# nevi-me/rust-dataframe

Measured on AMD Instinct MI355X. Metric: rows/sec filter+sum over 1e9 f64 Arrow rows; %HBM bw at 1/2/4/8 GPU, higher is better.
Workload: dtype f64

## Files before the change

rust_dataframe_amd/csrc/rdf_capi.cpp:

```cpp
#include <hip/hip_runtime.h>

#include <algorithm>
#include <cmath>
#include <cstdarg>
#include <cstdio>
#include <chrono>
#include <functional>
#include <cstring>
#include <map>
#include <memory>
#include <mutex>
#include <condition_variable>
#include <string>
#include <thread>
#include <vector>
#include <sys/syscall.h>
#include <unistd.h>

#include "rdf_device.h"
#include "rdf_stage_copy.h"

using namespace rdfk;

namespace {
// ... 54 lines not shown
    int    opt_gb_hot = 1;
    int    opt_gb_bucket = 0;
    int    opt_gb_partition = 3;
    bool   timing = false;
    std::vector<std::pair<hipEvent_t, hipEvent_t>> events;
    size_t events_used = 0;
    std::multimap<size_t, void*> pool_free;
    size_t pool_cached = 0;
    int64_t opt_stream_slab = 0;
    void*  sbuf_dev[2] = {nullptr, nullptr};
    void*  sbuf_pin[2] = {nullptr, nullptr};
    size_t sbuf_dev_cap = 0, sbuf_pin_cap = 0;
    hipEvent_t sbuf_ev[2] = {nullptr, nullptr};
    void*  dbuf_dev[2] = {nullptr, nullptr};
    void*  dbuf_pin[2] = {nullptr, nullptr};
    size_t dbuf_dev_cap = 0, dbuf_pin_cap = 0;
    hipEvent_t dbuf_ev[2] = {nullptr, nullptr};
    hipStream_t d2h_stream = nullptr;
    int64_t stream_slabs = 0, stream_bytes_staged = 0, stream_bytes_direct = 0;
    bool in_stream = false;
    bool streaming = false;
    int  opt_stream_table_kernel = 1;
    char* tab_pin = nullptr; size_t tab_pin_cap = 0, tab_pin_used = 0;
    bool   agg_comm_entered = false;
    ::rdf_comm* agg_comm = nullptr;
    ~Ctx();
};

thread_local Ctx g_ctx;

Ctx::~Ctx() {
    if (!ready || (long)syscall(SYS_gettid) == (long)getpid()) return;
    (void)hipSetDevice(device);
    if (stream) (void)hipStreamSynchronize(stream);
    for (void* p : arena.overflow) (void)hipFree(p);
    if (arena.base) (void)hipFree(arena.base);
    if (pinned) (void)hipHostFree(pinned);
    for (auto& kv : pool_free) (void)hipFree(kv.second);
    for (int b = 0; b < 2; ++b) { if (sbuf_dev[b]) (void)hipFree(sbuf_dev[b]); if (sbuf_pin[b]) (void)hipHostFree(sbuf_pin[b]); if (sbuf_ev[b]) (void)hipEventDestroy(sbuf_ev[b]); }
    if (tab_pin) (void)hipHostFree(tab_pin);
    if (d2h_stream) (void)hipStreamSynchronize(d2h_stream);
    for (int b = 0; b < 2; ++b) { if (dbuf_dev[b]) (void)hipFree(dbuf_dev[b]); if (dbuf_pin[b]) (void)hipHostFree(dbuf_pin[b]); if (dbuf_ev[b]) (void)hipEventDestroy(dbuf_ev[b]); }
    if (d2h_stream) (void)hipStreamDestroy(d2h_stream);
    for (auto& ev : events) { (void)hipEventDestroy(ev.first); (void)hipEventDestroy(ev.second); }
    if (copy_stream) { (void)hipStreamSynchronize(copy_stream); (void)hipStreamDestroy(copy_stream); }
    if (own_stream) (void)hipStreamDestroy(own_stream);
    ready = false;
}

rdf_status fail(rdf_status st, const char* fmt, ...) {
    char buf[512];
    va_list ap;
    va_start(ap, fmt);
    vsnprintf(buf, sizeof buf, fmt, ap);
    va_end(ap);
    g_ctx.err = buf;
    if (g_ctx.ready && g_ctx.stream) (void)hipStreamSynchronize(g_ctx.stream);
    return st;
}

// ... 834 lines not shown
                    static const int mir[6] = {LH_F_LT, LH_F_LE, LH_F_EQ, LH_F_NE, LH_F_GT, LH_F_GE};
                    h = (sw ? mir : fwd)[op - RDF_OP_GT];
                } else if (op == RDF_OP_AND) h = LH_AND;
                else if (op == RDF_OP_OR) h = LH_OR;
                else if (in.dtype == RDF_F64) {
                    if (op == RDF_OP_ADD) h = LH_F_ADD;
                    else if (op == RDF_OP_MUL) h = LH_F_MUL;
                    else if (op == RDF_OP_SUB) h = sw ? LH_F_RSUB : LH_F_SUB;
                    else if (op == RDF_OP_DIV) h = sw ? LH_F_RDIV : LH_F_DIV;
                } else if (in.dtype == RDF_I64 || in.dtype == RDF_U64) {
                    if (op == RDF_OP_ADD) h = LH_I_ADD;
                    else if (op == RDF_OP_MUL) h = LH_I_MUL;
                    else if (op == RDF_OP_SUB) h = sw ? LH_I_RSUB : LH_I_SUB;
                }
            } break;
            default: break;
        }
        if (h == LH_NONE) return false;
        lean.code[i].swapped = (uint8_t)((in.swapped & 1) | (h << 1));
    }
    return true;
}

rdf_status launch_agg_pair(const EvalArgs* ea, const FilterAggF64Args* fa, int cmp, int feat, int grid, int nvalues,
                           const int* cls, AggPartial* partials, AggPartial* result, const char* spec_sig = nullptr,
                           const SpecArgs* sa = nullptr) {
    Ctx& c = g_ctx;
    KernelTimer kt;
    if (sa) {
        const bool jit = jit_find(spec_sig) != nullptr;
        c.last_kernel = std::string("spec_kernel<") + spec_sig + ">" + (jit ? " [compiled at run time]" : "");
        const hipError_t le = launch_spec(spec_sig, *sa, grid, c.stream);
        if (le != hipSuccess && jit) { (void)hipGetLastError(); return kRetryInterpreted; }
        if (le != hipSuccess) return fail(RDF_DEVICE_ERROR, "launch_spec: %s", hipGetErrorString(le));
    }
    else if (fa) { c.last_kernel = "filter_agg_f64_kernel"; HIP_TRY(launch_filter_agg_f64(*fa, cmp, grid, c.stream)); }
    else {
        EvalArgs lean;
        if (c.opt_interp_lean && feat == 0 && lean_assign(*ea, lean)) { c.last_kernel = "eval_kernel<AGG, lean>"; HIP_TRY(launch_eval_lean(lean, SINK_AGG, grid, c.stream, c.opt_interp_lean == 2)); }
        else { c.last_kernel = "eval_kernel<AGG>"; HIP_TRY(launch_eval(*ea, SINK_AGG, feat, grid, c.stream)); }
    }
    kt.stop();
    AggFinalArgs f;
    memset(&f, 0, sizeof f);
    f.partials = partials;
    f.result = result;
    f.nblocks = grid;
    f.nvalues = nvalues;
    for (int k = 0; k < nvalues; ++k) f.value_cls[k] = cls[k];
    HIP_TRY(launch_agg_final(f, c.stream));
    return RDF_OK;
}

void fill_agg_result(rdf_agg_result* r, int dt, const AggPartial& p) {
    memset(r, 0, sizeof *r);
    r->dtype = dt;
    r->count = p.cnt;
    r->is_some = p.cnt > 0;
    if (is_float(dt)) {
        double s, a, b;
        memcpy(&s, &p.sum, 8); memcpy(&a, &p.mn, 8); memcpy(&b, &p.mx, 8);
        r->sum_f64 = dt == RDF_F32 ? (double)(float)s : s;
        if (p.cnt > 0) { r->min_f64 = a; r->max_f64 = b; }
    } else {
        r->sum_i64 = (int64_t)h_normalize_int(dt, p.sum);
        if (p.cnt > 0) { r->min_i64 = (int64_t)p.mn; r->max_i64 = (int64_t)p.mx; }
    }
}

}

struct rdf_frame {
    int device = 0;
// ... 285 lines not shown
            for (size_t i = 0; i < dev_outs.size(); ++i) dev_outs[i] = DevOutChunk{outs[i].values, outs[i].validity};
        }
    }

    std::vector<int64_t> tile_start;
    const rdf_frame::Tiles* eval_tiles = nullptr;
    if (fc) RDF_TRY(frame_tiles(*fc, kEvalTile, &eval_tiles));
    else {
        tile_start.assign((size_t)nchunks + 1, 0);
        for (int64_t c = 0; c < nchunks; ++c) tile_start[(size_t)c + 1] = tile_start[(size_t)c] + (clen[(size_t)c] + kEvalTile - 1) / kEvalTile;
    }
    const int64_t ntiles = fc ? eval_tiles->ntiles : tile_start[(size_t)nchunks];
    int grid = (int)(ntiles < (int64_t)eval_grid_limit() ? ntiles : (int64_t)eval_grid_limit());

    const size_t n_nc = ps.sink == RDF_SINK_STORE ? (size_t)ps.nvalues * (size_t)nchunks : 0;
    const int gwords = grouped ? group_words(ps.ngroups, ps.nvalues) : 0;
    const size_t scratch_bytes = 16 + n_nc * 8 + ((size_t)grid + 4) * (grouped ? (size_t)gwords * 8 : (size_t)ps.nvalues * sizeof(AggPartial));
    void* scratch = nullptr;
    RDF_TRY(arena_alloc(scratch_bytes, &scratch));
    uint32_t* d_flags = (uint32_t*)scratch;
    int64_t* d_nullc = (int64_t*)((char*)scratch + 16);
    AggPartial* d_partials = (AggPartial*)((char*)scratch + 16 + n_nc * 8);
    AggPartial* d_result = d_partials + (size_t)grid * (size_t)ps.nvalues;
    HIP_TRY(hipMemsetAsync(scratch, 0, 16 + n_nc * 8, ctx.stream));

    EvalArgs ea;
    memset(&ea, 0, sizeof ea);
    ea.nchunks = nchunks;
    ea.ntiles = ntiles;
    ea.ncols = ncols;
    ea.nvalues = ps.nvalues;
    ea.ncode = (int)cc.code.size();
    ea.ntmp = cc.tmp_max;
    ea.flags = d_flags;
    ea.out_null_counts = d_nullc;
    ea.partials = d_partials;
    for (int k = 0; k < ncols; ++k) ea.col_dtype[k] = col_dtype[k];
    int cls[kMaxGroupValues] = {0, 0, 0, 0, 0, 0, 0, 0};
    for (int v = 0; v < ps.nvalues; ++v) { cls[v] = value_class(value_dtype[v]); ea.value_cls[v] = cls[v]; }
    memcpy(ea.code, cc.code.data(), cc.code.size() * sizeof(Instr));

    TableBuilder tb;
    auto build_eval_tables = [&]() -> rdf_status {
        if (nchunks == 1) {
            for (int k = 0; k < ncols; ++k) ea.inline_cols[k] = in_dev[(size_t)k];
            for (int v = 0; v < ps.nvalues && ps.sink == RDF_SINK_STORE; ++v) ea.inline_outs[v] = dev_outs[(size_t)v];
            ea.inline_len = clen[0];
// ... 262 lines not shown
                if (L.kind == RDF_NODE_COLUMN && R.kind == RDF_NODE_SCALAR) { coln = &L; sc = &R; }
                else if (L.kind == RDF_NODE_SCALAR && R.kind == RDF_NODE_COLUMN) {
                    coln = &R; sc = &L;
                    cmp = fr.op == RDF_OP_GT ? RDF_OP_LT : fr.op == RDF_OP_GE ? RDF_OP_LE : fr.op == RDF_OP_LT ? RDF_OP_GT : fr.op == RDF_OP_LE ? RDF_OP_GE : fr.op;
                }
                if (coln && col_dtype[coln->column] == RDF_F64 && sc->dtype != RDF_NULLTYPE && (is_numeric(sc->dtype) || sc->dtype == RDF_BOOL)) {
                    const DevChunkCol& x = in_dev[(size_t)coln->column];
                    const DevChunkCol& y = in_dev[(size_t)vr.column];
                    const uintptr_t xa = (uintptr_t)((const double*)x.values + x.offset), ya = (uintptr_t)((const double*)y.values + y.offset);
                    if ((xa & 7) == 0 && (ya & 7) == 0 && (xa & 15) == (ya & 15)) {
                        memset(&fa, 0, sizeof fa);
                        fa.x = (const double*)x.values; fa.x_validity = x.validity; fa.x_offset = x.offset;
                        fa.y = (const double*)y.values; fa.y_validity = y.validity; fa.y_offset = y.offset;
                        fa.n = clen[0];
                        const uint64_t cu = cc.imm_for(*sc, RDF_F64);
                        memcpy(&fa.c, &cu, 8);
                        fa.partials = d_partials;
                        fast = true;
                    }
                }
            }
        }
        if (use_spec) {
            const rdf_status ls = launch_agg_pair(nullptr, nullptr, 0, 0, grid, ps.nvalues, cls, d_partials, d_result, sp.sig.c_str(), &sa);
            if (ls == kRetryInterpreted) return run_program(ps, cols, ncols, nchunks, outs, aggs, len_mismatch_msg, fc);
            RDF_TRY(ls);
        } else if (fast) {
            const int64_t per_block = (int64_t)kBlock * 4 * 2;
            int64_t want = (clen[0] + per_block - 1) / per_block;
            grid = (int)(want < (int64_t)eval_grid_limit() ? want : (int64_t)eval_grid_limit());
            if (grid < 1) grid = 1;
            d_result = d_partials + (size_t)grid * (size_t)ps.nvalues;
            RDF_TRY(launch_agg_pair(nullptr, &fa, cmp, 0, grid, 1, cls, d_partials, d_result));
        } else {
            RDF_TRY(launch_agg_pair(&ea, nullptr, 0, cc.feat(), grid, ps.nvalues, cls, d_partials, d_result));
        }
        if (ctx.agg_comm) {
            AggPartial hp[kMaxValues];
            uint32_t flags = 0;
            RDF_TRY(agg_dist_finish(*ctx.agg_comm, d_result, d_flags, ps.nvalues, cls, hp, &flags));
            if (flags & 2u) return fail(RDF_COMPUTE_ERROR, "pipeline_dist: another rank failed before the combine");
            if (flags & 1u) return fail(RDF_DIVIDE_BY_ZERO, "Divide by zero error");
            for (int v = 0; v < ps.nvalues; ++v) fill_agg_result(&aggs[v], value_dtype[v], hp[v]);
            return RDF_OK;
        }
        RDF_TRY(pinned_reserve(pin_off + 64 + sizeof(AggPartial) * kMaxValues));
        char* pin = ctx.pinned + pin_off;
        HIP_TRY(hipMemcpyAsync(pin, d_flags, 16, hipMemcpyDeviceToHost, ctx.stream));
        HIP_TRY(hipMemcpyAsync(pin + 64, d_result, sizeof(AggPartial) * (size_t)ps.nvalues, hipMemcpyDeviceToHost, ctx.stream));
        HIP_TRY(hipStreamSynchronize(ctx.stream));
        dbg.mark("kernel + result");
        uint32_t flags;
        memcpy(&flags, pin, 4);
        if (flags & 1u) return fail(RDF_DIVIDE_BY_ZERO, "Divide by zero error");
        for (int v = 0; v < ps.nvalues; ++v) {
            AggPartial p;
            memcpy(&p, pin + 64 + sizeof(AggPartial) * (size_t)v, sizeof p);
            fill_agg_result(&aggs[v], value_dtype[v], p);
        }
        return RDF_OK;
    }

    {
        KernelTimer kt;
        if (use_spec) {
            const bool jit = jit_find(sp.sig.c_str()) != nullptr;
            ctx.last_kernel = "spec_kernel<" + sp.sig + ">" + (jit ? " [compiled at run time]" : "");
            const hipError_t le = launch_spec(sp.sig.c_str(), sa, grid, ctx.stream);
            if (le != hipSuccess && jit) { (void)hipGetLastError(); return run_program(ps, cols, ncols, nchunks, outs, aggs, len_mismatch_msg, fc); }
            if (le != hipSuccess) return fail(RDF_DEVICE_ERROR, "launch_spec: %s", hipGetErrorString(le));
        }
        else {
            int64_t longest = 0;
            for (int64_t i = 0; i < nchunks; ++i) longest = std::max(longest, clen[(size_t)i]);
            EvalArgs lean;
            if (ctx.opt_interp_lean && cc.feat() == 0 && longest < ((int64_t)1 << 32) && lean_assign(ea, lean, SINK_STORE)) {
                ctx.last_kernel = "eval_kernel<STORE, lean>";
                HIP_TRY(launch_eval_lean(lean, SINK_STORE, grid, ctx.stream, ctx.opt_interp_lean == 2));
            } else { ctx.last_kernel = "eval_kernel<STORE>"; HIP_TRY(launch_eval(ea, SINK_STORE, cc.feat(), grid, ctx.stream)); }
        }
// ... 96 lines not shown
extern "C" {

const char* rdf_version(void) { return "rdf_mi355x 0.1.0 (gfx950)"; }
const char* rdf_last_error(void) { return g_ctx.err.c_str(); }

rdf_status rdf_device_count(int32_t* count) {
    if (!count) return fail(RDF_INVALID_ARGUMENT, "null pointer");
    int n = 0;
    hipError_t e = hipGetDeviceCount(&n);
    *count = e == hipSuccess ? n : 0;
    if (e != hipSuccess) return fail(RDF_DEVICE_ERROR, "hipGetDeviceCount: %s", hipGetErrorString(e));
    return RDF_OK;
}

rdf_status rdf_set_device(int32_t device) {
    Ctx& c = g_ctx;
    if (c.ready && c.device == device) return RDF_OK;
    if (c.ready) {
        (void)hipStreamSynchronize(c.stream);
        for (void* p : c.arena.overflow) (void)hipFree(p);
        c.arena.overflow.clear();
        if (c.arena.base) (void)hipFree(c.arena.base);
        c.arena = Arena();
        for (auto& ev : c.events) { (void)hipEventDestroy(ev.first); (void)hipEventDestroy(ev.second); }
        c.events.clear();
        c.events_used = 0;
        if (c.own_stream) (void)hipStreamDestroy(c.own_stream);
        c.own_stream = c.stream = nullptr;
        c.ready = false;
    }
    HIP_TRY(hipSetDevice(device));
    return ensure_ready();
}

rdf_status rdf_set_stream(void* hip_stream) {
    RDF_TRY(ensure_ready());
    g_ctx.stream = hip_stream ? (hipStream_t)hip_stream : g_ctx.own_stream;
    return RDF_OK;
}

rdf_status rdf_synchronize(void) {
    RDF_TRY(ensure_ready());
    HIP_TRY(hipStreamSynchronize(g_ctx.stream));
    return RDF_OK;
}

// ... 2505 lines not shown
```

rust_dataframe_amd/csrc/rdf_common.hip.h:

```cpp
#pragma once
#include "rdf_device.h"

namespace rdfk {

__device__ __forceinline__ uint64_t uniform64(uint64_t v) {
    uint32_t lo = __builtin_amdgcn_readfirstlane((uint32_t)v);
    uint32_t hi = __builtin_amdgcn_readfirstlane((uint32_t)(v >> 32));
    return ((uint64_t)hi << 32) | lo;
}
__device__ __forceinline__ int wave_id() { return __builtin_amdgcn_readfirstlane((int)(threadIdx.x >> 6)); }

template <class T> using GlobalPtr = const T __attribute__((address_space(1)))*;
template <class T> using GlobalMutPtr = T __attribute__((address_space(1)))*;
template <class T> __device__ __forceinline__ GlobalPtr<T> as_global(const void* p) { return (GlobalPtr<T>)p; }
template <class T> using ConstPtr = const T __attribute__((address_space(4)))*;
template <class T> __device__ __forceinline__ ConstPtr<T> as_const(const void* p) { return (ConstPtr<T>)p; }
__device__ __forceinline__ DevChunkCol const_col(const DevChunkCol* table, int64_t i) {
    const ConstPtr<DevChunkCol> t = as_const<DevChunkCol>(table);
    DevChunkCol c;
    c.values = t[i].values; c.validity = t[i].validity; c.offset = t[i].offset;
    return c;
}
template <class T> __device__ __forceinline__ GlobalMutPtr<T> as_global_mut(void* p) { return (GlobalMutPtr<T>)p; }

// ... 108 lines not shown
    cnt = 0;
    if (cls == CLS_F64) { sum = d2u(0.0); mn = mx = 0x7FF8000000000000ull; }
    else if (cls == CLS_SIGNED) { sum = 0; mn = (uint64_t)INT64_MAX; mx = (uint64_t)INT64_MIN; }
    else { sum = 0; mn = ~0ull; mx = 0; }
}
__device__ __forceinline__ void agg_merge(int cls, uint64_t& sum, uint64_t& mn, uint64_t& mx, int64_t& cnt,
                                          uint64_t s2, uint64_t mn2, uint64_t mx2, int64_t c2) {
    cnt += c2;
    if (cls == CLS_F64) {
        sum = d2u(u2d(sum) + u2d(s2));
        mn = d2u(fmin(u2d(mn), u2d(mn2)));
        mx = d2u(fmax(u2d(mx), u2d(mx2)));
    } else if (cls == CLS_SIGNED) {
        sum += s2;
        mn = (uint64_t)((int64_t)mn2 < (int64_t)mn ? (int64_t)mn2 : (int64_t)mn);
        mx = (uint64_t)((int64_t)mx2 > (int64_t)mx ? (int64_t)mx2 : (int64_t)mx);
    } else {
        sum += s2;
        mn = mn2 < mn ? mn2 : mn;
        mx = mx2 > mx ? mx2 : mx;
    }
}

__device__ __forceinline__ void block_reduce_agg(int cls, uint64_t sum, uint64_t mn, uint64_t mx, int64_t cnt,
                                                 AggPartial* lds4, AggPartial* out) {
#pragma unroll
    for (int m = 32; m >= 1; m >>= 1) {
        uint64_t s2 = shfl_xor64(sum, m), mn2 = shfl_xor64(mn, m), mx2 = shfl_xor64(mx, m);
        int64_t c2 = (int64_t)shfl_xor64((uint64_t)cnt, m);
        agg_merge(cls, sum, mn, mx, cnt, s2, mn2, mx2, c2);
    }
    const int wave = threadIdx.x >> 6;
    __syncthreads();
    if ((threadIdx.x & 63) == 0) { lds4[wave].sum = sum; lds4[wave].mn = mn; lds4[wave].mx = mx; lds4[wave].cnt = cnt; }
    __syncthreads();
    if (threadIdx.x == 0) {
        uint64_t s = lds4[0].sum, a = lds4[0].mn, b = lds4[0].mx;
        int64_t c = lds4[0].cnt;
        for (int w = 1; w < kBlock / 64; ++w) agg_merge(cls, s, a, b, c, lds4[w].sum, lds4[w].mn, lds4[w].mx, lds4[w].cnt);
        out->sum = s; out->mn = a; out->mx = b; out->cnt = c;
    }
}

__device__ __forceinline__ void trig_reduce(double x, double& r, int& q) {
    const double kd = rint(x * 6.36619772367581382433e-01);
    q = (int)kd;
    double t = fma(-kd, 1.57079632673412561417e+00, x);
    t = fma(-kd, 6.07710050630396597660e-11, t);
    t = fma(-kd, 2.02226624871116645580e-21, t);
    r = fma(-kd, 8.47842766036889956997e-32, t);
}
__device__ __forceinline__ double trig_ksin(double r) {
    const double z = r * r, v = z * r;
    const double p = fma(z, fma(z, fma(z, fma(z, 1.58969099521155010221e-10, -2.50507602534068634195e-08), 2.75573137070700676789e-06),
                                -1.98412698298579493134e-04), 8.33333333332248946124e-03);
    return fma(v, fma(z, p, -1.66666666666666324348e-01), r);
}
__device__ __forceinline__ double trig_kcos(double r) {
    const double z = r * r;
    const double p = z * fma(z, fma(z, fma(z, fma(z, fma(z, -1.13596475577881948265e-11, 2.08757232129817482790e-09), -2.75573143513906633035e-07),
                                            2.48015872894767294178e-05), -1.38888888888741095749e-03), 4.16666666666666019037e-02);
    return 1.0 - (0.5 * z - z * p);
}
// ... 214 lines not shown
```

rust_dataframe_amd/csrc/rdf_device.h:

```cpp
#pragma once
#include "rdf_sort_map.h"
#include <stdint.h>
#include <hip/hip_runtime.h>

#include <string>
#include "../../include/rdf_mi355x.h"

namespace rdfk {

constexpr int kBlock = 256;
constexpr int kVPT = 4;
constexpr int kEvalTile = kBlock * kVPT;
constexpr int kFilterTile = 4096;
constexpr int kFilterTileSmall = 1024;
constexpr int kMaxCode = 56;
constexpr int kMaxCols = 8;
constexpr int kMaxFrameCols = 64;
constexpr int kPreCols = 4;
constexpr int kMaxTmp = 4;
constexpr int kMaxValues = RDF_MAX_VALUES;
constexpr int kMaxGroupValues = RDF_MAX_GROUP_VALUES;
constexpr int kMaxFilterCols = 8;

struct DevChunkCol {
// ... 14 lines not shown
    uint8_t  op;
    uint8_t  dtype;
    uint8_t  src_kind;
    uint8_t  src_dtype;
    uint8_t  swapped;
    uint16_t src;
    uint64_t imm;
};
static_assert(sizeof(Instr) == 16, "Instr must stay 16 bytes");
enum : int {
    LH_NONE = 0, LH_LOAD, LH_STORE_TMP, LH_FILTER, LH_EMIT, LH_NOT, LH_CAST_I2F, LH_CAST_U2F,
    LH_F_GT, LH_F_GE, LH_F_EQ, LH_F_NE, LH_F_LT, LH_F_LE, LH_F_ADD, LH_F_SUB, LH_F_RSUB, LH_F_MUL, LH_F_DIV, LH_F_RDIV,
    LH_I_ADD, LH_I_SUB, LH_I_RSUB, LH_I_MUL, LH_AND, LH_OR
};

struct AggPartial {
    uint64_t sum, mn, mx;
    int64_t  cnt;
};
enum : int32_t { CLS_F64 = 0, CLS_SIGNED = 1, CLS_UNSIGNED = 2 };

enum : int32_t { SINK_STORE = 0, SINK_AGG = 1, SINK_GROUP = 2 };

struct EvalArgs {
    const DevChunkCol* cols;
    const int64_t*     chunk_tile_start;
    const int64_t*     chunk_len;
    DevOutChunk*       outs;
    int64_t*           out_null_counts;
    AggPartial*        partials;
    uint64_t*          group_partials;
    uint32_t*          flags;
    int64_t            nchunks, ntiles;
    DevChunkCol        inline_cols[kMaxCols];
    DevOutChunk        inline_outs[kMaxValues];
    int64_t            inline_len;
    int32_t            ncols, nvalues, ncode, ntmp;
    int32_t            col_dtype[kMaxCols];
    int32_t            value_cls[kMaxGroupValues];
    int32_t            ngroups, group_replicas;
    Instr              code[kMaxCode];
};

inline __host__ __device__ int group_words(int ngroups, int nvalues) { return (ngroups + 1) * (2 * nvalues + 1); }

constexpr int kGSpecCols = 8;
constexpr int kGSpecImm = 8;
struct GSpecArgs {
    const DevChunkCol* cols_tab;
    const int64_t*     chunk_tile_start;
    const int64_t*     chunk_len;
    DevChunkCol        cols[kGSpecCols];
    int32_t            col_map[kGSpecCols];
// ... 5 lines not shown
    int32_t            xcd_swz, tile_rot, pad1;
};

struct GroupFinalArgs {
    const uint64_t* partials;
    uint64_t*       result;
    int32_t         nblocks, words, ngroups, nvalues;
    int32_t         value_cls[kMaxGroupValues];
};

struct AggFinalArgs {
    const AggPartial* partials;
    AggPartial*       result;
    int32_t           nblocks, nvalues;
    int32_t           value_cls[kMaxValues];
};

struct FilterAggF64Args {
    const double*  x;   const uint8_t* x_validity;   int64_t x_offset;
    const double*  y;   const uint8_t* y_validity;   int64_t y_offset;
    int64_t        n;
    double         c;
    AggPartial*    partials;
};

constexpr int kSpecCols = 8;
constexpr int kSpecImm = 8;
struct SpecArgs {
    DevChunkCol        cols[kSpecCols];
    DevOutChunk        out;
    const DevChunkCol* cols_tab;
    const DevOutChunk* outs_tab;
    const int64_t*     chunk_tile_start;
    const int64_t*     chunk_len;
    int64_t            nchunks, ntiles;
    int64_t            n;
    uint64_t           tile_inv;
    uint64_t           imm[kSpecImm];
    int64_t*           out_null_count;
    AggPartial*        partials;
    uint32_t*          flags;
    int32_t            vec_bitmap;
    int32_t            rt[8];
    int32_t            alias[kSpecCols];
    int64_t            tile_rot;
    int32_t            xcd_swz, pad0;
};

struct MaskTables {
    const DevChunkCol* mask;
    const int64_t*     chunk_tile_start;
    const int64_t*     chunk_len;
    int64_t            nchunks, ntiles;
};
struct FilterArgs {
    MaskTables         t;
    const DevChunkCol* cols;
    DevOutChunk*       outs;
    int64_t*           out_null_counts;
    const int64_t*     tile_scan;
    int32_t            ncols;
    int32_t            esize[kMaxFilterCols];
};
// ... 543 lines not shown
```

rust_dataframe_amd/csrc/rdf_eval.hip:

```cpp
#include "rdf_common.hip.h"

#ifndef RDF_FEAT
#error "compile with -DRDF_FEAT=0|1|2"
#endif

namespace rdfk {


__device__ __forceinline__ uint64_t cast_value(int from, int to, uint64_t x, bool& ok) {
    ok = true;
    if (from == to) return x;
    double f = 0.0;
    bool src_float = false;
    if (from == RDF_F64) { f = u2d(x); src_float = true; }
    else if (from == RDF_F32) { f = (double)u2f(x); src_float = true; }
    if (to == RDF_BOOL) return src_float ? (uint64_t)(f != 0.0) : (uint64_t)(x != 0);
    if (to == RDF_F64) {
        if (src_float) return d2u(f);
        return d2u(dt_is_signed(from) ? (double)(int64_t)x : (double)x);
    }
    if (to == RDF_F32) {
        if (from == RDF_F64) return f2u((float)u2d(x));
        return f2u(dt_is_signed(from) ? (float)(int64_t)x : (float)x);
    }
// ... 656 lines not shown
    if (SINK == SINK_STORE && cur_chunk >= 0 && lane == 0) {
#pragma unroll
        for (int k = 0; k < NVAL; ++k)
            if (k < a.nvalues && nullacc[k])
                atomicAdd((unsigned long long*)&a.out_null_counts[(int64_t)k * a.nchunks + cur_chunk], (unsigned long long)nullacc[k]);
    }
    if (err) atomicOr(a.flags, err);
    if (SINK == SINK_GROUP) {
        __syncthreads();
        for (int w = tid; w < gwords; w += kBlock) {
            const bool fsum = w < a.nvalues * gS && a.value_cls[(w / gS) & (kMaxGroupValues - 1)] == CLS_F64;
            uint64_t acc0 = gtab[w];
            for (int r = 1; r < a.group_replicas; ++r) {
                const uint64_t x = gtab[(size_t)r * gwords + w];
                acc0 = fsum ? d2u(u2d(acc0) + u2d(x)) : acc0 + x;
            }
            a.group_partials[(size_t)blockIdx.x * gwords + w] = acc0;
        }
    }
    if (SINK == SINK_AGG) {
#pragma unroll
        for (int k = 0; k < NVAL; ++k)
            if (k < a.nvalues)
                block_reduce_agg(a.value_cls[k], g_sum[k], g_mn[k], g_mx[k], g_cnt[k], red_lds,
                                 &a.partials[(int64_t)blockIdx.x * a.nvalues + k]);
    }
}


template <int SINK, int NPRE, int NVAL>
static void launch_one(const EvalArgs& a, int grid, size_t lds, hipStream_t s) {
    hipLaunchKernelGGL((eval_kernel<RDF_FEAT, SINK, NPRE, NVAL>), dim3(grid), dim3(kBlock), lds, s, a);
}
template <int SINK>
static void launch_shape(const EvalArgs& a, int npre, int nval, int grid, size_t lds, hipStream_t s) {
    if (nval <= 1) {
        if (npre <= 1) launch_one<SINK, 1, 1>(a, grid, lds, s);
        else if (npre <= 2) launch_one<SINK, 2, 1>(a, grid, lds, s);
        else launch_one<SINK, 4, 1>(a, grid, lds, s);
    } else if (nval <= 2) {
        if (npre <= 2) launch_one<SINK, 2, 2>(a, grid, lds, s);
        else launch_one<SINK, 4, 2>(a, grid, lds, s);
    } else launch_one<SINK, 4, 4>(a, grid, lds, s);
}

#define RDF_CAT2(a, b) a##b
#define RDF_CAT(a, b) RDF_CAT2(a, b)
hipError_t RDF_CAT(launch_eval_feat, RDF_FEAT)(const EvalArgs& a, int sink, int grid, hipStream_t s) {
// ... 14 lines not shown
```

rust_dataframe_amd/csrc/rdf_eval_lean.hip:

```cpp
#include "rdf_common.hip.h"

namespace rdfk {

#define RDF_ROWS _Pragma("unroll") for (int j = 0; j < kVPT; ++j)

typedef uint64_t lean_u64x2 __attribute__((ext_vector_type(2)));
typedef uint32_t lean_u32x2 __attribute__((ext_vector_type(2)));

__device__ __forceinline__ uint32_t lean_nibble(const uint64_t (&w)[kVPT], int lane) {
    const uint32_t q = (uint32_t)lane >> 4, sh = ((uint32_t)lane & 15u) * 4u;
    const uint32_t c0 = (uint32_t)(w[0] >> sh), c1 = (uint32_t)(w[1] >> sh), c2 = (uint32_t)(w[2] >> sh), c3 = (uint32_t)(w[3] >> sh);
    const uint32_t m0 = 0u - (uint32_t)(q == 0), m1 = 0u - (uint32_t)(q == 1), m2 = 0u - (uint32_t)(q == 2), m3 = 0u - (uint32_t)(q == 3);
    return ((c0 & m0) | (c1 & m1) | (c2 & m2) | (c3 & m3)) & 15u;
}

__device__ __forceinline__ void lean_load8(const DevChunkCol cc, int64_t rw, int64_t clen, bool full, uint64_t (&v)[kVPT], uint32_t& valid) {
    const int lane = threadIdx.x & 63;
    const GlobalPtr<uint64_t> base = as_global<uint64_t>(cc.values) + cc.offset;
    if (full && (((uintptr_t)cc.values + (uintptr_t)(cc.offset + rw) * 8) & 15) == 0) {
        const GlobalPtr<lean_u64x2> p = (GlobalPtr<lean_u64x2>)(base + rw + (int64_t)lane * kVPT);
        const lean_u64x2 a0 = __builtin_nontemporal_load(p), a1 = __builtin_nontemporal_load(p + 1);
        v[0] = a0[0]; v[1] = a0[1]; v[2] = a1[0]; v[3] = a1[1];
    } else {
        const int64_t last = clen - 1;
// ... 46 lines not shown
        case LH_I_SUB: RDF_ROWS_R acc[r] = acc[r] - b(r); break;
        case LH_I_RSUB: RDF_ROWS_R acc[r] = b(r) - acc[r]; break;
        case LH_I_MUL: RDF_ROWS_R acc[r] = acc[r] * b(r); break;
        case LH_AND: RDF_ROWS_R acc[r] = acc[r] & b(r); break;
        default: RDF_ROWS_R acc[r] = acc[r] | b(r); break;
    }
}

__device__ __forceinline__ void lean_block_reduce(int cls, uint64_t sum, uint64_t mn, uint64_t mx, int64_t cnt, AggPartial* lds4, AggPartial* out) {
#pragma unroll
    for (int m = 32; m >= 1; m >>= 1) {
        const uint64_t s2 = shfl_xor64(sum, m), mn2 = shfl_xor64(mn, m), mx2 = shfl_xor64(mx, m);
        const int64_t c2 = (int64_t)shfl_xor64((uint64_t)cnt, m);
        agg_merge(cls, sum, mn, mx, cnt, s2, mn2, mx2, c2);
    }
    sum = uniform64(sum); mn = uniform64(mn); mx = uniform64(mx); cnt = (int64_t)uniform64((uint64_t)cnt);
    const int wave = wave_id();
    __syncthreads();
    lds4[wave].sum = sum; lds4[wave].mn = mn; lds4[wave].mx = mx; lds4[wave].cnt = cnt;
    __syncthreads();
    uint64_t s = lds4[0].sum, lo = lds4[0].mn, hi = lds4[0].mx;
    int64_t c = lds4[0].cnt;
    for (int w = 1; w < kBlock / 64; ++w) agg_merge(cls, s, lo, hi, c, lds4[w].sum, lds4[w].mn, lds4[w].mx, lds4[w].cnt);
    out->sum = s; out->mn = lo; out->mx = hi; out->cnt = c;
}

__device__ __forceinline__ void lean_store_words(uint8_t* bitmap, int64_t rw, int64_t rows_left, uint32_t nibble, int lane) {
    uint64_t x = (uint64_t)(nibble & 15u) << (((uint32_t)lane & 15u) * 4u);
#pragma unroll
    for (int m = 1; m < 16; m <<= 1) x |= shfl_xor64(x, m);
    const int64_t span = rows_left < 0 ? 0 : rows_left < (int64_t)kVPT * 64 ? rows_left : (int64_t)kVPT * 64;
    const int nwords = (int)((span + 63) >> 6);
    const __amdgpu_buffer_rsrc_t rs = __builtin_amdgcn_make_buffer_rsrc(bitmap + (rw >> 6) * 8, 0, nwords * 8, 0x00020000);
    lean_u32x2 w;
    w[0] = (uint32_t)x; w[1] = (uint32_t)(x >> 32);
    const uint32_t off = ((uint32_t)lane & 15u) == 0 ? ((uint32_t)lane >> 4) * 8u : 0x7FFFFFF0u;
    __builtin_amdgcn_raw_buffer_store_b64(w, rs, (int)off, 0, 0);
}

template <int SINK, int NPRE, int NVAL, int T>
__global__ __launch_bounds__(kBlock) void eval_lean_kernel(const EvalArgs a) {
    constexpr int R = T * kVPT;
    constexpr uint32_t kAllRows = (1u << R) - 1u;
    extern __shared__ __attribute__((aligned(16))) unsigned char smem[];
    __shared__ AggPartial red_lds[kBlock / 64];
    const int tid = threadIdx.x, lane = tid & 63;
    const int wave = wave_id();
// ... 222 lines not shown
                        uint64_t opnd[R];
                        uint32_t opv = 0;
                        if (kind == SRC_COL) {
#pragma unroll
                            for (int p = 0; p < NPRE; ++p)
                                if (p == src) { opv = colvalid[p]; RDF_ROWS_R opnd[r] = colv[r / kVPT][p][r % kVPT]; }
                            if (sdt == RDF_I64) RDF_ROWS_R opnd[r] = d2u((double)(int64_t)opnd[r]);
                            else RDF_ROWS_R opnd[r] = d2u((double)opnd[r]);
                        } else {
                            const uint64_t* tv = tmp_vals + (size_t)src * R * kBlock + tid;
                            RDF_ROWS_R opnd[r] = tv[r * kBlock];
                            opv = tmp_valid[src * kBlock + tid];
                        }
                        accv &= opv;
                        lean_bin<R>(h, acc, [&](int r) { return opnd[r]; }, accv & inr, err);
                    }
                } break;
            }
        }
        tile = ntile;
        have = nhave;
    }

    if (__ballot(err != 0) != 0) *(volatile uint32_t*)a.flags = 1u;
    if constexpr (SINK == SINK_AGG) {
#pragma unroll
        for (int k = 0; k < NVAL; ++k)
            if (k < a.nvalues)
                lean_block_reduce(a.value_cls[k], g_sum[k], g_mn[k], g_mx[k], g_cnt[k], red_lds, &a.partials[(int64_t)blockIdx.x * a.nvalues + k]);
    }
}

template <int SINK, int NPRE, int NVAL, int T>
static void lean_launch_one(const EvalArgs& a, int grid, hipStream_t s) {
    const size_t lds = (size_t)a.ntmp * ((size_t)T * kVPT * kBlock * 8 + kBlock * 4);
    hipLaunchKernelGGL((eval_lean_kernel<SINK, NPRE, NVAL, T>), dim3(grid), dim3(kBlock), lds, s, a);
}

hipError_t launch_eval_lean(const EvalArgs& a, int sink, int grid, hipStream_t s, bool one_tile) {
    const int npre = a.ncols, nval = a.nvalues;
    const bool two = !one_tile && (npre <= 1 || (npre <= 2 && sink == SINK_AGG)) && (size_t)a.ntmp * (2 * kVPT * kBlock * 8 + kBlock * 4) <= 65536;
    if (sink == SINK_STORE) {
        if (npre <= 1) { if (two) lean_launch_one<SINK_STORE, 1, 1, 2>(a, grid, s); else lean_launch_one<SINK_STORE, 1, 1, 1>(a, grid, s); }
        else if (npre <= 2) lean_launch_one<SINK_STORE, 2, 1, 1>(a, grid, s);
        else lean_launch_one<SINK_STORE, 4, 1, 1>(a, grid, s);
    } else if (nval <= 1) {
        if (npre <= 1) { if (two) lean_launch_one<SINK_AGG, 1, 1, 2>(a, grid, s); else lean_launch_one<SINK_AGG, 1, 1, 1>(a, grid, s); }
        else if (npre <= 2) { if (two) lean_launch_one<SINK_AGG, 2, 1, 2>(a, grid, s); else lean_launch_one<SINK_AGG, 2, 1, 1>(a, grid, s); }
        else lean_launch_one<SINK_AGG, 4, 1, 1>(a, grid, s);
    } else if (nval <= 2) {
        if (npre <= 2) { if (two) lean_launch_one<SINK_AGG, 2, 2, 2>(a, grid, s); else lean_launch_one<SINK_AGG, 2, 2, 1>(a, grid, s); }
        else lean_launch_one<SINK_AGG, 4, 2, 1>(a, grid, s);
// ... 6 lines not shown
```

rust_dataframe_amd/csrc/rdf_kernels.hip:

```cpp
#include "rdf_common.hip.h"
#include "rdf_join_place.h"

namespace rdfk {

__global__ __launch_bounds__(kBlock) void agg_final_kernel(const AggFinalArgs a) {
    __shared__ AggPartial red_lds[kBlock / 64];
    for (int k = 0; k < a.nvalues; ++k) {
        const int cls = a.value_cls[k];
        uint64_t s, mn, mx;
        int64_t cnt;
        agg_init(cls, s, mn, mx, cnt);
        for (int b = threadIdx.x; b < a.nblocks; b += kBlock) {
            const AggPartial p = a.partials[(int64_t)b * a.nvalues + k];
            agg_merge(cls, s, mn, mx, cnt, p.sum, p.mn, p.mx, p.cnt);
        }
        block_reduce_agg(cls, s, mn, mx, cnt, red_lds, &a.result[k]);
        __syncthreads();
    }
}


template <int CMP>
__device__ __forceinline__ bool cmp_f64(double x, double c) {
    if (CMP == RDF_OP_GT) return x > c;
    if (CMP == RDF_OP_GE) return x >= c;
    if (CMP == RDF_OP_EQ) return x == c;
    if (CMP == RDF_OP_NE) return x != c;
    if (CMP == RDF_OP_LT) return x < c;
    return x <= c;
}

struct F64Agg {
    double sum, mn, mx;
    int64_t cnt;
    __device__ __forceinline__ void init() { sum = 0.0; mn = mx = __longlong_as_double(0x7FF8000000000000ll); cnt = 0; }
    __device__ __forceinline__ void add(double v) { sum += v; mn = fmin(mn, v); mx = fmax(mx, v); ++cnt; }
};

constexpr int kFU = 4;
typedef double dvec2 __attribute__((ext_vector_type(2)));

// ... 41 lines not shown
                if (!SAME) vy[u] = (dvec2)(0.0);
            }
        }
        uint64_t wx[2 * kFU], wy[2 * kFU];
        if (HASV) {
            const int64_t rw = 2 * wbase;
            if (a.x_validity) load_windows<2 * kFU>(a.x_validity, a.x_offset + head + rw, body_rows - rw, wx);
            if (!SAME && a.y_validity) load_windows<2 * kFU>(a.y_validity, a.y_offset + head + rw, body_rows - rw, wy);
        }
#pragma unroll
        for (int u = 0; u < kFU; ++u) {
            const int64_t i = wbase + u * 64 + lane;
            uint32_t bits = i < nvec ? 3u : 0u;
            if (HASV) {
                const int sh = (2 * lane) & 63;
                if (a.x_validity) bits &= (uint32_t)((lane < 32 ? wx[2 * u] : wx[2 * u + 1]) >> sh) & 3u;
                if (!SAME && a.y_validity) bits &= (uint32_t)((lane < 32 ? wy[2 * u] : wy[2 * u + 1]) >> sh) & 3u;
            }
            const dvec2 yy = SAME ? vx[u] : vy[u];
            if ((bits & 1u) && cmp_f64<CMP>(vx[u].x, a.c)) g.add(yy.x);
            if ((bits & 2u) && cmp_f64<CMP>(vx[u].y, a.c)) g.add(yy.y);
        }
    }
    block_reduce_agg(CLS_F64, d2u(g.sum), d2u(g.mn), d2u(g.mx), g.cnt, red_lds, &a.partials[blockIdx.x]);
}

template <int WW> constexpr int filter_tile_rows() { return WW * 64 * (kBlock / 64); }
static_assert(filter_tile_rows<16>() == kFilterTile && filter_tile_rows<4>() == kFilterTileSmall, "tile sizes of the two instantiations");

template <int WW>
__device__ __forceinline__ void locate_tile(const MaskTables& t, int64_t tile, int64_t& c, int64_t& r0, int64_t& clen) {
    c = t.nchunks == 1 ? 0 : find_chunk_tile(t.chunk_tile_start, t.nchunks, tile);
    r0 = (tile - t.chunk_tile_start[c]) * filter_tile_rows<WW>();
    clen = t.chunk_len[c];
}

template <int kWW>
__device__ __forceinline__ void keep_words(const DevChunkCol& m, int64_t rw, int64_t clen, uint64_t (&kw)[kWW]) {
    load_windows<kWW>((const uint8_t*)m.values, m.offset + rw, clen - rw, kw);
    if (m.validity) {
        uint64_t vw[kWW];
        load_windows<kWW>(m.validity, m.offset + rw, clen - rw, vw);
#pragma unroll
        for (int i = 0; i < kWW; ++i) kw[i] &= vw[i];
    }
}

// ... 1752 lines not shown
```

rust_dataframe_amd/csrc/rdf_spec_kernel.hip.h:

```cpp
#pragma once
#include <map>
#include <string>
#include <type_traits>

#include "rdf_expr.hip.h"

namespace rdfk {


template <int DT> struct AggT;
template <> struct AggT<RDF_F64> {
    double sum, mn, mx; int64_t cnt;
    static constexpr int cls = CLS_F64;
    __device__ __forceinline__ void init() { sum = 0.0; mn = mx = __longlong_as_double(0x7FF8000000000000ll); cnt = 0; }
    __device__ __forceinline__ void add(double v) { sum += v; mn = fmin(mn, v); mx = fmax(mx, v); ++cnt; }
    __device__ __forceinline__ uint64_t s() const { return d2u(sum); }
    __device__ __forceinline__ uint64_t a() const { return d2u(mn); }
    __device__ __forceinline__ uint64_t b() const { return d2u(mx); }
};
template <> struct AggT<RDF_I64> {
    uint64_t sum; int64_t mn, mx; int64_t cnt;
    static constexpr int cls = CLS_SIGNED;
    __device__ __forceinline__ void init() { sum = 0; mn = INT64_MAX; mx = INT64_MIN; cnt = 0; }
    __device__ __forceinline__ void add(int64_t v) { sum += (uint64_t)v; mn = v < mn ? v : mn; mx = v > mx ? v : mx; ++cnt; }
// ... 395 lines not shown
#pragma unroll
                        for (int e = 0; e < RV; ++e) if ((inu >> e) & 1) as_global_mut<So>(out.values)[(int64_t)RV * i + e] = (So)x[e];
                    }
                }
                if (out.validity) {
#pragma unroll
                    for (int h = 0; h < RV; ++h) {
                        const uint64_t wv = interleave_word<RV>(vb, h, lane);
                        if (lane == RV * u + h) word_vld = wv;
                    }
                }
#pragma unroll
                for (int e = 0; e < RV; ++e) nulls += (uint32_t)__popcll(inb[e] & ~vb[e]);
            }
            if (lane < R && rw + 64 * lane < n) {
                if constexpr (V0::dt == RDF_BOOL) as_global_mut<uint64_t>(out.values)[(rw >> 6) + lane] = word_val;
                if (out.validity) as_global_mut<uint64_t>(out.validity)[(rw >> 6) + lane] = word_vld;
            }
        }
    }
    if (c.err) atomicOr(a.flags, c.err);
    if constexpr (P::SINK == SINK_AGG) {
        constexpr int nv = has_v1 ? 2 : 1;
        block_reduce_agg(g0.cls, g0.s(), g0.a(), g0.b(), g0.cnt, red_lds, &a.partials[(int64_t)blockIdx.x * nv]);
        if constexpr (has_v1) block_reduce_agg(g1.cls, g1.s(), g1.a(), g1.b(), g1.cnt, red_lds, &a.partials[(int64_t)blockIdx.x * nv + 1]);
    } else {
        if (cur_chunk >= 0 && lane == 0 && nulls) atomicAdd((unsigned long long*)&a.out_null_count[cur_chunk], (unsigned long long)nulls);
    }
}


typedef void (*SpecLaunch)(const SpecArgs&, int, hipStream_t);
struct SpecEntry { SpecLaunch launch; int rows_per_tile; };
std::map<std::string, SpecEntry>& spec_registry();

template <class P>
static void launch_prog(const SpecArgs& a, int grid, hipStream_t s) {
    hipLaunchKernelGGL((spec_kernel<P>), dim3(grid), dim3(kBlock), 0, s, a);
}
template <class P>
static void reg() { spec_registry()[P::sig()] = SpecEntry{&launch_prog<P>, 64 * P::R}; }

struct Lc; struct Lk;
template <int FROM> struct Lx;
template <class X, class Y> struct Op;
template <class X> struct Tr;
template <class Sh, int S, int C, int K, int DT> struct Build;
template <int S, int C, int K, int DT> struct Build<Lc, S, C, K, DT> {
// ... 111 lines not shown
```

Measured before the change: 846.6 billion.

## Fuse final aggregate reduction into main kernel via last-block completion counter

Removes the separate agg_final_kernel launch: each block publishes its partial with agent-scope atomics, and the last block to finish (found through sharded atomic counters in a persistent device state buffer) folds all partials. It writes the result and flags directly into a pinned host record, which replaces the device-to-host memcpys and the flags memset. This cuts launch, copy and sync overhead per query. In exchange it adds counter contention, a spin-wait in the last block and a cross-scope memory-ordering subtlety.

```diff
diff --git a/rust_dataframe_amd/csrc/rdf_capi.cpp b/rust_dataframe_amd/csrc/rdf_capi.cpp
--- a/rust_dataframe_amd/csrc/rdf_capi.cpp
+++ b/rust_dataframe_amd/csrc/rdf_capi.cpp
@@ -100,6 +100,8 @@
     bool streaming = false;
     int  opt_stream_table_kernel = 1;
     char* tab_pin = nullptr; size_t tab_pin_cap = 0, tab_pin_used = 0;
+    uint32_t* agg_state = nullptr;
+    char*     agg_record = nullptr;
     bool   agg_comm_entered = false;
     ::rdf_comm* agg_comm = nullptr;
     ~Ctx();
@@ -114,6 +116,8 @@
     for (void* p : arena.overflow) (void)hipFree(p);
     if (arena.base) (void)hipFree(arena.base);
     if (pinned) (void)hipHostFree(pinned);
+    if (agg_state) (void)hipFree(agg_state);
+    if (agg_record) (void)hipHostFree(agg_record);
     for (auto& kv : pool_free) (void)hipFree(kv.second);
     for (int b = 0; b < 2; ++b) { if (sbuf_dev[b]) (void)hipFree(sbuf_dev[b]); if (sbuf_pin[b]) (void)hipHostFree(sbuf_pin[b]); if (sbuf_ev[b]) (void)hipEventDestroy(sbuf_ev[b]); }
     if (tab_pin) (void)hipHostFree(tab_pin);
@@ -994,10 +998,36 @@
     return true;
 }
 
-rdf_status launch_agg_pair(const EvalArgs* ea, const FilterAggF64Args* fa, int cmp, int feat, int grid, int nvalues,
-                           const int* cls, AggPartial* partials, AggPartial* result, const char* spec_sig = nullptr,
-                           const SpecArgs* sa = nullptr) {
+rdf_status agg_tail_ready() {
     Ctx& c = g_ctx;
+    if (!c.agg_record) {
+        void* p = nullptr;
+        const hipError_t e = hipHostMalloc(&p, 4096, hipHostMallocDefault);
+        if (e != hipSuccess) return fail(RDF_MEMORY_ERROR, "hipHostMalloc(4096) for the aggregate record failed: %s", hipGetErrorString(e));
+        c.agg_record = (char*)p;
+    }
+    if (!c.agg_state) {
+        void* p = nullptr;
+        HIP_TRY(hipMalloc(&p, kAggStateBytes));
+        c.agg_state = (uint32_t*)p;
+        HIP_TRY(hipMemsetAsync(p, 0, kAggStateBytes, c.stream));
+        HIP_TRY(hipStreamSynchronize(c.stream));
+    }
+    return RDF_OK;
+}
+
+rdf_status launch_agg_pair(EvalArgs* ea, FilterAggF64Args* fa, int cmp, int feat, int grid, AggPartial* result, uint32_t* flags_out,
+                           const char* spec_sig = nullptr, SpecArgs* sa = nullptr) {
+    Ctx& c = g_ctx;
+    RDF_TRY(agg_tail_ready());
+    AggTail t;
+    t.state = c.agg_state;
+    t.flags_out = flags_out;
+    t.result = result;
+    t.record = c.agg_record;
+    if (sa) { sa->agg_tail = t; sa->flags = c.agg_state + kAggFlagsWord; }
+    else if (fa) fa->agg_tail = t;
+    else { ea->agg_tail = t; ea->flags = c.agg_state + kAggFlagsWord; }
     KernelTimer kt;
     if (sa) {
         const bool jit = jit_find(spec_sig) != nullptr;
@@ -1013,14 +1043,6 @@
         else { c.last_kernel = "eval_kernel<AGG>"; HIP_TRY(launch_eval(*ea, SINK_AGG, feat, grid, c.stream)); }
     }
     kt.stop();
-    AggFinalArgs f;
-    memset(&f, 0, sizeof f);
-    f.partials = partials;
-    f.result = result;
-    f.nblocks = grid;
-    f.nvalues = nvalues;
-    for (int k = 0; k < nvalues; ++k) f.value_cls[k] = cls[k];
-    HIP_TRY(launch_agg_final(f, c.stream));
     return RDF_OK;
 }
 
@@ -1352,7 +1374,7 @@
     int64_t* d_nullc = (int64_t*)((char*)scratch + 16);
     AggPartial* d_partials = (AggPartial*)((char*)scratch + 16 + n_nc * 8);
     AggPartial* d_result = d_partials + (size_t)grid * (size_t)ps.nvalues;
-    HIP_TRY(hipMemsetAsync(scratch, 0, 16 + n_nc * 8, ctx.stream));
+    if (ps.sink != RDF_SINK_AGG) HIP_TRY(hipMemsetAsync(scratch, 0, 16 + n_nc * 8, ctx.stream));
 
     EvalArgs ea;
     memset(&ea, 0, sizeof ea);
@@ -1661,7 +1683,7 @@
             }
         }
         if (use_spec) {
-            const rdf_status ls = launch_agg_pair(nullptr, nullptr, 0, 0, grid, ps.nvalues, cls, d_partials, d_result, sp.sig.c_str(), &sa);
+            const rdf_status ls = launch_agg_pair(nullptr, nullptr, 0, 0, grid, d_result, d_flags, sp.sig.c_str(), &sa);
             if (ls == kRetryInterpreted) return run_program(ps, cols, ncols, nchunks, outs, aggs, len_mismatch_msg, fc);
             RDF_TRY(ls);
         } else if (fast) {
@@ -1670,9 +1692,9 @@
             grid = (int)(want < (int64_t)eval_grid_limit() ? want : (int64_t)eval_grid_limit());
             if (grid < 1) grid = 1;
             d_result = d_partials + (size_t)grid * (size_t)ps.nvalues;
-            RDF_TRY(launch_agg_pair(nullptr, &fa, cmp, 0, grid, 1, cls, d_partials, d_result));
+            RDF_TRY(launch_agg_pair(nullptr, &fa, cmp, 0, grid, d_result, d_flags));
         } else {
-            RDF_TRY(launch_agg_pair(&ea, nullptr, 0, cc.feat(), grid, ps.nvalues, cls, d_partials, d_result));
+            RDF_TRY(launch_agg_pair(&ea, nullptr, 0, cc.feat(), grid, d_result, d_flags));
         }
         if (ctx.agg_comm) {
             AggPartial hp[kMaxValues];
@@ -1683,18 +1705,15 @@
             for (int v = 0; v < ps.nvalues; ++v) fill_agg_result(&aggs[v], value_dtype[v], hp[v]);
             return RDF_OK;
         }
-        RDF_TRY(pinned_reserve(pin_off + 64 + sizeof(AggPartial) * kMaxValues));
-        char* pin = ctx.pinned + pin_off;
-        HIP_TRY(hipMemcpyAsync(pin, d_flags, 16, hipMemcpyDeviceToHost, ctx.stream));
-        HIP_TRY(hipMemcpyAsync(pin + 64, d_result, sizeof(AggPartial) * (size_t)ps.nvalues, hipMemcpyDeviceToHost, ctx.stream));
         HIP_TRY(hipStreamSynchronize(ctx.stream));
         dbg.mark("kernel + result");
+        const char* rec = ctx.agg_record;
         uint32_t flags;
-        memcpy(&flags, pin, 4);
+        memcpy(&flags, rec, 4);
         if (flags & 1u) return fail(RDF_DIVIDE_BY_ZERO, "Divide by zero error");
         for (int v = 0; v < ps.nvalues; ++v) {
             AggPartial p;
-            memcpy(&p, pin + 64 + sizeof(AggPartial) * (size_t)v, sizeof p);
+            memcpy(&p, rec + kAggRecordValues + sizeof(AggPartial) * (size_t)v, sizeof p);
             fill_agg_result(&aggs[v], value_dtype[v], p);
         }
         return RDF_OK;
@@ -1837,6 +1856,8 @@
         c.arena.overflow.clear();
         if (c.arena.base) (void)hipFree(c.arena.base);
         c.arena = Arena();
+        if (c.agg_state) (void)hipFree(c.agg_state);
+        c.agg_state = nullptr;
         for (auto& ev : c.events) { (void)hipEventDestroy(ev.first); (void)hipEventDestroy(ev.second); }
         c.events.clear();
         c.events_used = 0;
diff --git a/rust_dataframe_amd/csrc/rdf_common.hip.h b/rust_dataframe_amd/csrc/rdf_common.hip.h
--- a/rust_dataframe_amd/csrc/rdf_common.hip.h
+++ b/rust_dataframe_amd/csrc/rdf_common.hip.h
@@ -154,8 +154,22 @@
     }
 }
 
+enum : int { AGG_ST_PLAIN = 0, AGG_ST_AGENT = 1, AGG_ST_SYSTEM = 2 };
+template <int ST>
+__device__ __forceinline__ void store_partial(AggPartial* p, uint64_t s, uint64_t a, uint64_t b, int64_t c) {
+    if constexpr (ST == AGG_ST_PLAIN) { p->sum = s; p->mn = a; p->mx = b; p->cnt = c; }
+    else {
+        constexpr int scope = ST == AGG_ST_AGENT ? __HIP_MEMORY_SCOPE_AGENT : __HIP_MEMORY_SCOPE_SYSTEM;
+        __hip_atomic_store(&p->sum, s, __ATOMIC_RELAXED, scope);
+        __hip_atomic_store(&p->mn, a, __ATOMIC_RELAXED, scope);
+        __hip_atomic_store(&p->mx, b, __ATOMIC_RELAXED, scope);
+        __hip_atomic_store(&p->cnt, c, __ATOMIC_RELAXED, scope);
+    }
+}
+
+template <int ST = AGG_ST_PLAIN>
 __device__ __forceinline__ void block_reduce_agg(int cls, uint64_t sum, uint64_t mn, uint64_t mx, int64_t cnt,
-                                                 AggPartial* lds4, AggPartial* out) {
+                                                 AggPartial* lds4, AggPartial* out, AggPartial* out2 = nullptr) {
 #pragma unroll
     for (int m = 32; m >= 1; m >>= 1) {
         uint64_t s2 = shfl_xor64(sum, m), mn2 = shfl_xor64(mn, m), mx2 = shfl_xor64(mx, m);
@@ -170,7 +184,58 @@
         uint64_t s = lds4[0].sum, a = lds4[0].mn, b = lds4[0].mx;
         int64_t c = lds4[0].cnt;
         for (int w = 1; w < kBlock / 64; ++w) agg_merge(cls, s, a, b, c, lds4[w].sum, lds4[w].mn, lds4[w].mx, lds4[w].cnt);
-        out->sum = s; out->mn = a; out->mx = b; out->cnt = c;
+        store_partial<ST>(out, s, a, b, c);
+        if (out2) store_partial<AGG_ST_SYSTEM>(out2, s, a, b, c);
+    }
+}
+
+__device__ __forceinline__ void agg_fold(const AggPartial* partials, int nblocks, int nvalues, uint32_t cls_bits, AggPartial* lds4,
+                                         AggPartial* out, AggPartial* out2 = nullptr) {
+    nvalues = __builtin_amdgcn_readfirstlane(nvalues);
+    for (int k = 0; k < nvalues; ++k) {
+        const int cls = __builtin_amdgcn_readfirstlane((int)((cls_bits >> (2 * k)) & 3u));
+        uint64_t s, mn, mx;
+        int64_t cnt;
+        agg_init(cls, s, mn, mx, cnt);
+#pragma nounroll
+        for (int b = threadIdx.x; b < nblocks; b += kBlock) {
+            const AggPartial p = partials[(int64_t)b * nvalues + k];
+            agg_merge(cls, s, mn, mx, cnt, p.sum, p.mn, p.mx, p.cnt);
+        }
+        block_reduce_agg(cls, s, mn, mx, cnt, lds4, &out[k], out2 ? &out2[k] : nullptr);
+        __syncthreads();
+    }
+}
+
+__device__ __forceinline__ void agg_finish(const AggTail& t, const AggPartial* partials, int nvalues, uint32_t cls_bits, AggPartial* lds4) {
+    uint32_t* const st = t.state;
+    const uint32_t g = gridDim.x, nshard = g < 8u ? g : 8u;
+    asm volatile("s_waitcnt vmcnt(0)" ::: "memory");
+    __syncthreads();
+    if (threadIdx.x == 0) {
+        uint32_t last = 0;
+        const uint32_t s = blockIdx.x & 7u;
+        if (__hip_atomic_fetch_add(st + s * kAggLineWords, 1u, __ATOMIC_RELAXED, __HIP_MEMORY_SCOPE_AGENT) + 1u == (g - s + 7u) >> 3)
+            last = __hip_atomic_fetch_add(st + kAggFullWord, 1u, __ATOMIC_RELAXED, __HIP_MEMORY_SCOPE_AGENT) + 1u == nshard;
+        if (last) {
+            for (uint32_t k = 0; k < nshard; ++k)
+                while (__hip_atomic_load(st + k * kAggLineWords, __ATOMIC_RELAXED, __HIP_MEMORY_SCOPE_AGENT) != (g - k + 7u) >> 3) {}
+            __builtin_amdgcn_fence(__ATOMIC_ACQUIRE, "agent");
+            asm volatile("s_waitcnt vmcnt(0)" ::: "memory");
+        }
+        reinterpret_cast<volatile uint32_t*>(lds4)[0] = last;
+    }
+    __syncthreads();
+    if (__builtin_amdgcn_readfirstlane(reinterpret_cast<volatile uint32_t*>(lds4)[0]) == 0) return;
+    AggPartial* const rec = reinterpret_cast<AggPartial*>(t.record + kAggRecordValues);
+    agg_fold(partials, (int)g, nvalues, cls_bits, lds4, t.result, rec);
+    if (threadIdx.x == 0) {
+        const uint32_t f = __hip_atomic_exchange(st + kAggFlagsWord, 0u, __ATOMIC_RELAXED, __HIP_MEMORY_SCOPE_AGENT);
+        for (uint32_t k = 0; k < nshard; ++k) __hip_atomic_store(st + k * kAggLineWords, 0u, __ATOMIC_RELAXED, __HIP_MEMORY_SCOPE_AGENT);
+        __hip_atomic_store(st + kAggFullWord, 0u, __ATOMIC_RELAXED, __HIP_MEMORY_SCOPE_AGENT);
+        t.flags_out[0] = f; t.flags_out[1] = 0; t.flags_out[2] = 0; t.flags_out[3] = 0;
+        __hip_atomic_store(reinterpret_cast<uint32_t*>(t.record), f, __ATOMIC_RELAXED, __HIP_MEMORY_SCOPE_SYSTEM);
+        asm volatile("s_waitcnt vmcnt(0)" ::: "memory");
     }
 }
 
diff --git a/rust_dataframe_amd/csrc/rdf_device.h b/rust_dataframe_amd/csrc/rdf_device.h
--- a/rust_dataframe_amd/csrc/rdf_device.h
+++ b/rust_dataframe_amd/csrc/rdf_device.h
@@ -60,6 +60,18 @@
 
 enum : int32_t { SINK_STORE = 0, SINK_AGG = 1, SINK_GROUP = 2 };
 
+constexpr int kAggLineWords = 32;
+constexpr int kAggFullWord = 8 * kAggLineWords;
+constexpr int kAggFlagsWord = 9 * kAggLineWords;
+constexpr int kAggStateBytes = 10 * kAggLineWords * 4;
+constexpr int kAggRecordValues = 64;
+struct AggTail {
+    uint32_t*   state;
+    uint32_t*   flags_out;
+    AggPartial* result;
+    char*       record;
+};
+
 struct EvalArgs {
     const DevChunkCol* cols;
     const int64_t*     chunk_tile_start;
@@ -67,6 +79,7 @@
     DevOutChunk*       outs;
     int64_t*           out_null_counts;
     AggPartial*        partials;
+    AggTail            agg_tail;
     uint64_t*          group_partials;
     uint32_t*          flags;
     int64_t            nchunks, ntiles;
@@ -118,6 +131,7 @@
     int64_t        n;
     double         c;
     AggPartial*    partials;
+    AggTail        agg_tail;
 };
 
 constexpr int kSpecCols = 8;
@@ -135,6 +149,7 @@
     uint64_t           imm[kSpecImm];
     int64_t*           out_null_count;
     AggPartial*        partials;
+    AggTail            agg_tail;
     uint32_t*          flags;
     int32_t            vec_bitmap;
     int32_t            rt[8];
diff --git a/rust_dataframe_amd/csrc/rdf_eval.hip b/rust_dataframe_amd/csrc/rdf_eval.hip
--- a/rust_dataframe_amd/csrc/rdf_eval.hip
+++ b/rust_dataframe_amd/csrc/rdf_eval.hip
@@ -702,8 +702,11 @@
 #pragma unroll
         for (int k = 0; k < NVAL; ++k)
             if (k < a.nvalues)
-                block_reduce_agg(a.value_cls[k], g_sum[k], g_mn[k], g_mx[k], g_cnt[k], red_lds,
-                                 &a.partials[(int64_t)blockIdx.x * a.nvalues + k]);
+                block_reduce_agg<AGG_ST_AGENT>(a.value_cls[k], g_sum[k], g_mn[k], g_mx[k], g_cnt[k], red_lds,
+                                               &a.partials[(int64_t)blockIdx.x * a.nvalues + k]);
+        uint32_t cls_bits = 0;
+        for (int k = 0; k < a.nvalues; ++k) cls_bits |= (uint32_t)a.value_cls[k] << (2 * k);
+        agg_finish(a.agg_tail, a.partials, a.nvalues, cls_bits, red_lds);
     }
 }
 
diff --git a/rust_dataframe_amd/csrc/rdf_eval_lean.hip b/rust_dataframe_amd/csrc/rdf_eval_lean.hip
--- a/rust_dataframe_amd/csrc/rdf_eval_lean.hip
+++ b/rust_dataframe_amd/csrc/rdf_eval_lean.hip
@@ -92,7 +92,11 @@
     uint64_t s = lds4[0].sum, lo = lds4[0].mn, hi = lds4[0].mx;
     int64_t c = lds4[0].cnt;
     for (int w = 1; w < kBlock / 64; ++w) agg_merge(cls, s, lo, hi, c, lds4[w].sum, lds4[w].mn, lds4[w].mx, lds4[w].cnt);
-    out->sum = s; out->mn = lo; out->mx = hi; out->cnt = c;
+    store_partial<AGG_ST_AGENT>(out, s, lo, hi, c);
+}
+
+__device__ __noinline__ void lean_agg_finish(const AggTail t, const AggPartial* partials, int nvalues, uint32_t cls_bits, AggPartial* lds4) {
+    agg_finish(t, partials, nvalues, cls_bits, lds4);
 }
 
 __device__ __forceinline__ void lean_store_words(uint8_t* bitmap, int64_t rw, int64_t rows_left, uint32_t nibble, int lane) {
@@ -361,12 +365,16 @@
         have = nhave;
     }
 
-    if (__ballot(err != 0) != 0) *(volatile uint32_t*)a.flags = 1u;
+    if (__ballot(err != 0) != 0) __hip_atomic_store(a.flags, 1u, __ATOMIC_RELAXED, __HIP_MEMORY_SCOPE_AGENT);
     if constexpr (SINK == SINK_AGG) {
 #pragma unroll
         for (int k = 0; k < NVAL; ++k)
             if (k < a.nvalues)
                 lean_block_reduce(a.value_cls[k], g_sum[k], g_mn[k], g_mx[k], g_cnt[k], red_lds, &a.partials[(int64_t)blockIdx.x * a.nvalues + k]);
+        uint32_t cls_bits = 0;
+#pragma unroll
+        for (int k = 0; k < NVAL; ++k) cls_bits |= k < a.nvalues ? (uint32_t)a.value_cls[k] << (2 * k) : 0u;
+        lean_agg_finish(a.agg_tail, a.partials, a.nvalues, cls_bits, red_lds);
     }
 }
 
diff --git a/rust_dataframe_amd/csrc/rdf_kernels.hip b/rust_dataframe_amd/csrc/rdf_kernels.hip
--- a/rust_dataframe_amd/csrc/rdf_kernels.hip
+++ b/rust_dataframe_amd/csrc/rdf_kernels.hip
@@ -5,18 +5,9 @@
 
 __global__ __launch_bounds__(kBlock) void agg_final_kernel(const AggFinalArgs a) {
     __shared__ AggPartial red_lds[kBlock / 64];
-    for (int k = 0; k < a.nvalues; ++k) {
-        const int cls = a.value_cls[k];
-        uint64_t s, mn, mx;
-        int64_t cnt;
-        agg_init(cls, s, mn, mx, cnt);
-        for (int b = threadIdx.x; b < a.nblocks; b += kBlock) {
-            const AggPartial p = a.partials[(int64_t)b * a.nvalues + k];
-            agg_merge(cls, s, mn, mx, cnt, p.sum, p.mn, p.mx, p.cnt);
-        }
-        block_reduce_agg(cls, s, mn, mx, cnt, red_lds, &a.result[k]);
-        __syncthreads();
-    }
+    uint32_t cls_bits = 0;
+    for (int k = 0; k < a.nvalues; ++k) cls_bits |= (uint32_t)a.value_cls[k] << (2 * k);
+    agg_fold(a.partials, a.nblocks, a.nvalues, cls_bits, red_lds, a.result);
 }
 
 
@@ -104,7 +95,8 @@
             if ((bits & 2u) && cmp_f64<CMP>(vx[u].y, a.c)) g.add(yy.y);
         }
     }
-    block_reduce_agg(CLS_F64, d2u(g.sum), d2u(g.mn), d2u(g.mx), g.cnt, red_lds, &a.partials[blockIdx.x]);
+    block_reduce_agg<AGG_ST_AGENT>(CLS_F64, d2u(g.sum), d2u(g.mn), d2u(g.mx), g.cnt, red_lds, &a.partials[blockIdx.x]);
+    agg_finish(a.agg_tail, a.partials, 1, CLS_F64, red_lds);
 }
 
 template <int WW> constexpr int filter_tile_rows() { return WW * 64 * (kBlock / 64); }
diff --git a/rust_dataframe_amd/csrc/rdf_spec_kernel.hip.h b/rust_dataframe_amd/csrc/rdf_spec_kernel.hip.h
--- a/rust_dataframe_amd/csrc/rdf_spec_kernel.hip.h
+++ b/rust_dataframe_amd/csrc/rdf_spec_kernel.hip.h
@@ -441,8 +441,9 @@
     if (c.err) atomicOr(a.flags, c.err);
     if constexpr (P::SINK == SINK_AGG) {
         constexpr int nv = has_v1 ? 2 : 1;
-        block_reduce_agg(g0.cls, g0.s(), g0.a(), g0.b(), g0.cnt, red_lds, &a.partials[(int64_t)blockIdx.x * nv]);
-        if constexpr (has_v1) block_reduce_agg(g1.cls, g1.s(), g1.a(), g1.b(), g1.cnt, red_lds, &a.partials[(int64_t)blockIdx.x * nv + 1]);
+        block_reduce_agg<AGG_ST_AGENT>(g0.cls, g0.s(), g0.a(), g0.b(), g0.cnt, red_lds, &a.partials[(int64_t)blockIdx.x * nv]);
+        if constexpr (has_v1) block_reduce_agg<AGG_ST_AGENT>(g1.cls, g1.s(), g1.a(), g1.b(), g1.cnt, red_lds, &a.partials[(int64_t)blockIdx.x * nv + 1]);
+        agg_finish(a.agg_tail, a.partials, nv, (uint32_t)g0.cls | (has_v1 ? (uint32_t)g1.cls << 2 : 0u), red_lds);
     } else {
         if (cur_chunk >= 0 && lane == 0 && nulls) atomicAdd((unsigned long long*)&a.out_null_count[cur_chunk], (unsigned long long)nulls);
     }
```

Result: no change. 841.0 billion (median of 6 runs) (-0.7%).
